# hkbharath/MARL-MASS

Measured on AMD Instinct MI355X. Metric: agent-steps/sec (whole node), MASS CBF shield on, 65536 envs x 8 CAVs, higher is better.
Workload: dtype f64

## Files before the change

marl-mass_amd/csrc/mm_kernels.hip:

```cpp
#include <hip/hip_runtime.h>
#include <math.h>
#include <stdio.h>
#include <string.h>

#include <type_traits>

#include "mm_device.h"
#include "mm_div.h"
#include "mm_handle.h"
#define MM_COUNTS_FN __host__ __device__ inline
#include "../../include/mm_counts.h"

using namespace mm;

struct DevCfg {
  int env_kind, shield, nsub, T, action_masking, auto_reset, obs_f64, N, E, debug_flags, n_hdv;
  double dt, collision_reward, high_speed_reward, headway_cost, headway_time, merging_lane_cost;
  double rs_lo, rs_hi, eta, tau;
  double inv_dt, rs_span, rs_ispan, rs_span2, rs_ispan2;
  int agent_reward;
  int steer_vel;
  int *err;
  int traffic_density, mixed_traffic, num_cav;
};
constexpr int kMetricsAccBit = 30;
#define MM_LATCH_QP_BOUNDS 1
#define MM_LATCH_BAD_ACTION 2
#define MM_LATCH_BAD_QP 4
#define MM_LATCH_INTERNAL 8
enum { MM_LW_STEP = 0, MM_LW_QP = 1, MM_LW_SHIELD = 2, MM_LW_COUNT = 3 };
struct DevState {
  double *F;
  uint8_t *B;
  int32_t *I;
  uint64_t *seeds;
  long long A;
  int E, N;
};

enum {
  SW_CPSI, SW_ACCN,
  SW_AX, SW_AY, SW_AH, SW_ACPSI, SW_AGVX, SW_ASTEER, SW_ASPSI,
  SW_BX, SW_BY, SW_BH, SW_BCPSI, SW_BGVX, SW_BSTEER, SW_BSPSI,
  SW_ACC,
  SW_F_COUNT
};
enum { SW_WPK, SW_APK, SW_BPK, SW_META, SW_RES, SW_CLS, SW_I_COUNT };
struct SweepBuf {
  double *F;
  int *I;
  uint8_t *order;
  uint8_t *envf;
  uint8_t *urgent;
  long long Ep;
  int N;
};
MM_DEV double &sw_f(const SweepBuf &sb, int f, int a, long long e) { return sb.F[((long long)f * sb.N + a) * sb.Ep + e]; }
MM_DEV int &sw_i(const SweepBuf &sb, int f, int a, long long e) { return sb.I[((long long)f * sb.N + a) * sb.Ep + e]; }

#ifndef MM_TU
#define MM_TU 0
#endif

#ifdef MM_STAMPS
#define MM_STAMP_WAVES (1 << 16)
__device__ unsigned long long g_stamps_w[MM_STAMP_WAVES * 16];
__device__ unsigned long long g_stamps_s[4096 * 8];
#define SSTAMP(k)                                                                        \
  do {                                                                                   \
    unsigned long long _t = __builtin_amdgcn_s_memtime();                                \
    if ((threadIdx.x & 63) == (k)) _t_acc += _t - _t_last;                               \
    _t_last = __builtin_amdgcn_s_memtime();                                              \
  } while (0)
#define SCOUNT(k) do { if ((threadIdx.x & 63) == (k)) _t_acc += 1; } while (0)
#define STAMP(k)                                                                         \
  do {                                                                                   \
    unsigned long long _t = __builtin_amdgcn_s_memtime();                                \
    if ((threadIdx.x & 63) == (k)) _t_acc += _t - _t_last;                               \
    _t_last = __builtin_amdgcn_s_memtime();                                              \
  } while (0)
#else
#define STAMP(k) do {} while (0)
#define SSTAMP(k) do {} while (0)
#define SCOUNT(k) do {} while (0)
#endif

template <int KIND> constexpr bool kIdm = KIND == MM_ENV_HDV_V1;

struct Veh {
  double x, y, h, v, tspeed;
  double act_steer, act_acc, safe_steer, safe_acc, gvx;
  double h1x, h1vx, h2x, h2vx;
  double sang;
  int lane, tlane, sidx, crashed, hl, flags, hist_len;
  int kind;
  bool present;
};

MM_DEV int lane_id() { return threadIdx.x & 63; }
MM_DEV double shfl_d(double v, int src) { return __shfl(v, src, 64); }
MM_DEV int shfl_i(int v, int src) { return __shfl(v, src, 64); }

template <int M>
MM_DEV int dppx_i(int v) {
  static_assert(M >= 1 && M <= 15, "xor mask within a 16-lane DPP row");
  if constexpr (M == 1) return __builtin_amdgcn_update_dpp(0, v, 0xB1, 0xF, 0xF, false);
  else if constexpr (M == 2) return __builtin_amdgcn_update_dpp(0, v, 0x4E, 0xF, 0xF, false);
  else if constexpr (M == 3) return __builtin_amdgcn_update_dpp(0, v, 0x1B, 0xF, 0xF, false);
  else if constexpr (M == 7) return __builtin_amdgcn_update_dpp(0, v, 0x141, 0xF, 0xF, false);
  else if constexpr (M == 8) return __builtin_amdgcn_update_dpp(0, v, 0x128, 0xF, 0xF, false);
  else if constexpr (M == 15) return __builtin_amdgcn_update_dpp(0, v, 0x140, 0xF, 0xF, false);
// ... 1036 lines not shown
      if (redo) {
#ifdef MM_STAMPS
        atomicAdd(&g_stamps_s[blockIdx.x % 4096 * 8 + 6], 1ull);
#endif
        s_redo[ln] = 0;
        reload_views();
        r = 0; dirty = (c.debug_flags & 1) != 0; nospec = true;
        phase = PH_SETUP;
      }
      continue;
    }
    if (__any(phase == PH_RUN)) {
      if (phase == PH_RUN) sing = mm_qp_bottom(&q, &rs) == 0;
    }
    SSTAMP(3);
  }
  if (e < c.E) sb.urgent[e] = slow_now ? 1 : 0;
#ifdef MM_STAMPS
  if ((threadIdx.x & 63) < 8 && blockIdx.x < 4096) g_stamps_s[blockIdx.x * 8 + (threadIdx.x & 63)] += _t_acc;
#endif
}

#ifndef MM_MIN_WAVES
#define MM_MIN_WAVES 2
#endif
#ifndef MM_NONE_WAVES
#define MM_NONE_WAVES 3
#endif
#ifndef MM_NONE_WIDE_G
#define MM_NONE_WIDE_G 99
#endif
#ifndef MM_IPM_WAVES
#define MM_IPM_WAVES 2
#endif
#ifndef MM_IPM_CAV_WAVES
#define MM_IPM_CAV_WAVES 2
#endif
#ifndef MM_IPM_WIDE_WAVES
#define MM_IPM_WIDE_WAVES 1
#endif
#ifndef MM_SPLIT_WAVES
#define MM_SPLIT_WAVES 2
#endif
template <int G, int SHIELD, bool MIXED>
#ifndef MM_GENERAL_NONE_WAVES
#define MM_GENERAL_NONE_WAVES 3
#endif
constexpr int step_min_waves(bool ipm = false) { return SHIELD == MM_SHIELD_NONE ? (G >= MM_NONE_WIDE_G ? 2 : (MIXED ? MM_GENERAL_NONE_WAVES : MM_NONE_WAVES)) : (ipm ? (G >= 6 ? MM_IPM_WIDE_WAVES : (MIXED ? MM_IPM_WAVES : MM_IPM_CAV_WAVES)) : MM_MIN_WAVES); }
template <int G, int KIND, int SHIELD, bool MIXED, bool IPM = false, bool TRACE = false, bool SPLIT = false>
#ifndef MM_STEP_BLOCK
#define MM_STEP_BLOCK 64
#endif
__global__ __launch_bounds__(MM_STEP_BLOCK, (SPLIT ? MM_SPLIT_WAVES : step_min_waves<G, SHIELD, MIXED>(IPM))) void step_kernel(DevCfg c, DevState st, const int32_t *__restrict__ actions,
                                                   MMStepOut out, double *metrics, SweepBuf sb, int kb) {
  constexpr bool IDM = kIdm<KIND>;
  constexpr bool LC = (KIND == MM_ENV_V1) || IDM;
  constexpr bool SHIELDED = LC && (SHIELD != MM_SHIELD_NONE);
  static_assert(!IDM || (MIXED && SHIELD == MM_SHIELD_NONE && !IPM && !SPLIT), "hdv-v1: general unshielded kernels only");
  constexpr bool MASS = (SHIELD == MM_SHIELD_MASS);
  static_assert(!IPM || SHIELDED, "the IPM mode lives in shielded kernels");
  static_assert(!SPLIT || IPM, "the split form exists for the interior-point kernels");
#ifdef MM_SERIAL_ALL
  constexpr bool kSerialOnly = true || IPM;
#else
#ifdef MM_SERIAL_MASS
  constexpr bool kSerialOnly = MIXED || MASS || IPM;
#else
  constexpr bool kSerialOnly = MIXED;
#endif
#endif
  constexpr bool kSine = SHIELDED && !SPLIT && !MIXED && !IPM && !kSerialOnly && kPow2<G> && G <= 8;
  static_assert(kPow2<G> || MM_STEP_BLOCK == 64, "rotation layouts: one wave per workgroup");
  const long long gtid = (long long)blockIdx.x * blockDim.x + threadIdx.x;
  constexpr int kTail = kPow2<G> ? 64 : (64 / G) * G;
  const bool tail = lane_id() >= kTail;
  const int gb = kPow2<G> ? (lane_id() & ~(G - 1)) : (tail ? kTail - G : lane_id() - lane_id() % G);
  const int a = kPow2<G> ? (int)(gtid % G) : lane_id() - gb;
  const long long e = kPow2<G> ? gtid / G : (tail ? (long long)st.E : (gtid >> 6) * (64 / G) + lane_id() / G);
  const bool valid = e < st.E && a < st.N;
  const long long i = e * st.N + a;
  const long long A = st.A;
  const double dt = c.dt;

#ifdef MM_STAMPS
  unsigned long long _t_last = __builtin_amdgcn_s_memtime(), _t_acc = 0;
#endif
  Veh v;
  const bool sv = MIXED && KIND == MM_ENV_V1 && c.steer_vel != 0;
  load_veh(st, i, valid, v, sv);
  int steps = 0, time = 0, n_merge = 0, episode = 0;
  if (e < st.E) {
    steps = st.I[MM_E_STEPS * st.E + e]; time = st.I[MM_E_TIME * st.E + e];
  }
  if (!MIXED && v.kind == 2) v.kind = 1;
  if (IDM && v.present) v.kind = 2;
  const bool hdv = MIXED && v.kind == 2;
  const bool ctrl = IDM ? v.present : (v.present && !hdv);
  const bool ctrl_x = IDM ? false : ctrl;
  int action = (!IDM && valid && ctrl) ? actions[i] : 1;
  if ((unsigned)action > 4u) {
    if (!SPLIT || kb == 0) atomicOr(c.err, MM_LATCH_BAD_ACTION);
    action = 1;
  }
  const unsigned present_bits = group_ballot<G>(v.present, gb);
  const unsigned ctrl_bits = group_ballot<G>(ctrl, gb);
  const int n_veh = __popc(present_bits), n_ctrl = __popc(ctrl_bits);
  if (!SPLIT || kb == 0) steps += 1;

  double cpsi = 1.0, spsi = 0.0;
  double st_t = __builtin_nan("");
  if (v.present) mmm_sincos(v.h, &spsi, &cpsi);
  int pk_self = v.lane;
  if (SHIELDED && v.present) pk_self = pose_code(v.lane, next_lane(v.lane, v.x, v.y), MASS ? corner_flags(v.x, v.y, spsi, cpsi, v.lane) : 0);

  enum { C_B = 0, C_H1X = 8, C_H1VX, C_H2X, C_H2VX, C_SSTEER, C_SACC, C_TSPEED, C_A = 15, C_GU0 = 23, C_GU1 = 24, C_PRE = 25, C_MSGW = 29 };
  constexpr bool kMailbox = G <= 8 || !kPow2<G>;
  constexpr bool kPackMsg = !kPow2<G>;
  constexpr int kColdB = kMailbox ? (kPackMsg ? 29 : 30) : 25;
  constexpr bool kRoomy = false;
  constexpr int C_CPSI = kColdB + G - 1, C_GVX = C_CPSI + 1;
  constexpr int kColdN = !SHIELDED ? 15 : (kSerialOnly ? 23 : kColdB + G - 1 + (kRoomy ? 2 : 0));
  static_assert(kColdN * MM_STEP_BLOCK * 8 >= (MM_STEP_BLOCK / 64) * 64 * 30 * 4, "the obs staging must fit in the cold slots");
  __shared__ double s_cold[kColdN][MM_STEP_BLOCK];
  const int tid = threadIdx.x;
  auto cold_i = [&](int slot, int col) -> int & { return ((int *)&s_cold[slot][col])[0]; };
  if (LC) {
    s_cold[C_H1X][tid] = v.h1x; s_cold[C_H1VX][tid] = v.h1vx; s_cold[C_H2X][tid] = v.h2x; s_cold[C_H2VX][tid] = v.h2vx;
    s_cold[C_SSTEER][tid] = v.safe_steer; s_cold[C_SACC][tid] = v.safe_acc;
  }
  s_cold[C_TSPEED][tid] = v.tspeed;
  if constexpr (kRoomy) { s_cold[C_CPSI][tid] = cpsi; s_cold[C_GVX][tid] = v.gvx; }
  auto CPSI = [&]() -> double { if constexpr (kRoomy) return s_cold[C_CPSI][tid]; else return cpsi; };
  auto GVX = [&]() -> double { if constexpr (kRoomy) return s_cold[C_GVX][tid]; else return v.gvx; };
  bool env_active = IDM ? n_veh > 0 : n_ctrl > 0;
  if constexpr (SPLIT) {
    if (kb > 0) env_active = e < st.E && sb.envf[e] != 0;
  }
  STAMP(0);
  const int k_lo = SPLIT ? (kb > 0 ? kb - 1 : 0) : 0, k_hi = SPLIT ? (kb < c.nsub ? kb : c.nsub - 1) : c.nsub - 1;
  for (int k = k_lo; k <= k_hi; k++) {
    const bool head = !SPLIT || k == kb, tail = !SPLIT || k != kb;
    const bool live = env_active && v.present;
    QpTrace qt = {0, __builtin_nan(""), __builtin_nan(""), __builtin_nan(""), __builtin_nan(""),
                  __builtin_nan(""), __builtin_nan(""), __builtin_nan("")};
    int rank = 0;
    if ((SHIELDED || MIXED) && head) {
      for_partners<G>([&](auto mc) {
        constexpr int m = decltype(mc)::value;
        double px = px_d<m, G>(v.x, a);
        bool pp = px_i<m, G>((int)live, a) != 0;
        rank += (pp && (px > v.x || (px == v.x && pidx<m, G>(a) < a))) ? 1 : 0;
      });
    }
    if (head) v.tspeed = s_cold[C_TSPEED][tid];
    if (live && !hdv && head) {
      if (time % c.nsub == 0) hl_act<KIND>(v, action);
    }
    const int tl_pre = v.tlane;
    if (live && !hdv && head) controlled_act<!MIXED, kSine>(v, -1, sv, st_t);
    if (head) s_cold[C_TSPEED][tid] = v.tspeed;
    if constexpr (MIXED) { STAMP(1); }
    if constexpr (MIXED) {
      if (head && __any(hdv && live)) {
        const bool acting = hdv && live && !v.crashed;
        double koff = 0.0, koff_obst = 0.0;
        if (__any(acting && v.lane == MM_LANE_KB0)) {
// ... 772 lines not shown
  }
  if (valid) {
    if (out.agents_rewards) out.agents_rewards[i] = ctrl ? local : 0;
    if (out.regional_rewards) out.regional_rewards[i] = ctrl ? regional : 0;
    if (out.agents_dones) out.agents_dones[i] = ctrl ? (uint8_t)(v.crashed || steps >= c.T || v.x < 0) : 1;
    if (out.crashed) out.crashed[i] = v.present ? (uint8_t)v.crashed : 0;
    if (out.agents_info) {
      out.agents_info[i * 3 + 0] = v.present ? v.x : 0;
      out.agents_info[i * 3 + 1] = v.present ? v.y : 0;
      out.agents_info[i * 3 + 2] = v.present ? v.v : 0;
    }
  }
  if (e < st.E && a == 0 && env_ok) {
    if (out.reward) out.reward[e] = reward;
    if (out.done) out.done[e] = (uint8_t)done;
    if (out.average_speed) out.average_speed[e] = avg_speed;
    if (out.traffic_speed) out.traffic_speed[e] = traffic_speed;
    if (out.min_headway) out.min_headway[e] = min_headway;
    if (out.merge_percent) out.merge_percent[e] = merge_pct;
  }
  STAMP(10);
  if (metrics) {
    static_assert(MM_STEP_BLOCK % 64 == 0, "whole waves per workgroup");
    const bool lead = e < st.E && a == 0 && env_ok;
    const double mv[8] = {lead ? reward : 0.0, (lead && done && crashed_bits) ? 1.0 : 0.0, lead ? avg_speed : 0.0,
                          lead ? traffic_speed : 0.0, lead ? 1.0 : 0.0, (lead && done) ? merge_pct : 0.0,
                          (lead && done) ? 1.0 : 0.0, lead ? min_headway : INFINITY};
    if (a == 0) {
#pragma unroll
      for (int k = 0; k < 8; k++) s_cold[C_B + k][tid] = mv[k];
    }
    __builtin_amdgcn_fence(__ATOMIC_RELEASE, "wavefront");
    __builtin_amdgcn_wave_barrier();
    __builtin_amdgcn_fence(__ATOMIC_ACQUIRE, "wavefront");
    const int ln = lane_id();
    if (ln < 8) {
      const int slot = C_B + ln, base = tid - ln;
      double acc = ln == 7 ? INFINITY : 0.0;
#pragma unroll
      for (int j = 0; j < 64 / G; j++) {
        const double x = s_cold[slot][base + j * G];
        acc = ln == 7 ? fmin(acc, x) : acc + x;
      }
      double *row = metrics + (gtid >> 6) * 8;
      if ((c.debug_flags >> kMetricsAccBit) & 1) {
        if (ln == 7) (void)unsafeAtomicMin(&row[7], acc);
        else (void)unsafeAtomicAdd(&row[ln], acc);
      } else {
        row[ln] = acc;
      }
    }
  }
  STAMP(15);
  if (c.auto_reset && done) {
    const uint64_t seed = st.seeds[e];
    Veh nv;
    memset(&nv, 0, sizeof nv);
    int nm = 0;
    int nc = n_ctrl, nh = n_veh - n_ctrl;
    if constexpr (IDM) { nc = 0; nh = n_veh; }
    episode_counts<KIND>(c, seed, (uint32_t)episode, nc, nh);
    const bool spawn = valid && (c.traffic_density > 0 ? a < nc + nh : v.present);
    if (spawn) nm = spawn_vehicle(nv, a, nc, nh, seed, (uint32_t)episode);
    if (c.traffic_density > 0 && valid) {
      if (!spawn) {
        if (v.present) {
          Veh z;
          memset(&z, 0, sizeof z);
          store_veh(st, i, z, true);
        }
        v.present = false; v.kind = 0;
      }
      st.B[MM_B_KIND * A + i] = spawn ? (uint8_t)nv.kind : (uint8_t)0;
    }
    if (spawn) {
      v = nv;
      spsi = 0.0; cpsi = 1.0;
      s_cold[C_H1X][tid] = v.h1x; s_cold[C_H1VX][tid] = v.h1vx; s_cold[C_H2X][tid] = v.h2x; s_cold[C_H2VX][tid] = v.h2vx;
      s_cold[C_SSTEER][tid] = v.safe_steer; s_cold[C_SACC][tid] = v.safe_acc; s_cold[C_TSPEED][tid] = v.tspeed;
    }
    n_merge = shfl_i(nm, gb);
    steps = 0; time = 0; episode += 1;
  }
  if (valid && v.present) {
    if (LC) {
      v.h1x = s_cold[C_H1X][tid]; v.h1vx = s_cold[C_H1VX][tid]; v.h2x = s_cold[C_H2X][tid]; v.h2vx = s_cold[C_H2VX][tid];
      if (!hdv) { v.safe_steer = s_cold[C_SSTEER][tid]; v.safe_acc = s_cold[C_SACC][tid]; }
    }
    v.tspeed = s_cold[C_TSPEED][tid];
    store_veh(st, i, v, sv);
  }
  if (e < st.E && a == 0) {
    st.I[MM_E_STEPS * st.E + e] = steps; st.I[MM_E_TIME * st.E + e] = time;
    st.I[MM_E_N_MERGE * st.E + e] = n_merge; st.I[MM_E_EPISODE * st.E + e] = episode;
  }
  STAMP(11);
  __syncthreads();
  STAMP(14);
  const double sc_h[2] = {spsi, cpsi};
  observe<G, KIND, true>(c, v, a, gb, i, valid, out.obs, out.action_mask, (float *)&s_cold[0][0], sc_h);
  STAMP(12);
#ifdef MM_STAMPS
  {
    const long long wv = gtid >> 6;
    if ((threadIdx.x & 63) < 16 && wv < MM_STAMP_WAVES) g_stamps_w[wv * 16 + (threadIdx.x & 63)] += _t_acc;
  }
#endif
}

template <int G, int KIND>
__global__ __launch_bounds__(256) void reset_kernel(DevCfg c, DevState st, int mode, const uint8_t *env_mask,
                                                    const uint64_t *seeds_in, void *obs, uint8_t *avail) {
  const long long gtid = (long long)blockIdx.x * blockDim.x + threadIdx.x;
  const long long e = gtid / G;
  const int a = (int)(gtid % G);
  const int gb = lane_id() & ~(G - 1);
  const bool valid = e < st.E && a < st.N;
  const long long i = e * st.N + a;
  const bool selected = e < st.E && mode != 2 && (!env_mask || env_mask[e]);
  Veh v;
  load_veh(st, i, valid, v);
  if (kIdm<KIND> && v.present) v.kind = 2;
  if (selected) {
    int steps = 0, time = 0, n_merge = 0, episode = st.I[MM_E_EPISODE * st.E + e];
    if (mode == 0) {
      if (seeds_in && a == 0) st.seeds[e] = seeds_in[e];
      const uint64_t seed = seeds_in ? seeds_in[e] : st.seeds[e];
      int nm = 0;
      int nc = st.N - c.n_hdv, nh = c.n_hdv;
      if (kIdm<KIND>) { nc = 0; nh = st.N; }
      episode_counts<KIND>(c, seed, (uint32_t)episode, nc, nh);
      if (valid) {
        if (a < nc + nh) nm = spawn_vehicle(v, a, nc, nh, seed, (uint32_t)episode);
        else {
          const bool was = v.present;
          memset(&v, 0, sizeof v);
          if (was) store_veh(st, i, v, true);
          v.hl = MM_HL_NONE;
        }
        st.B[MM_B_KIND * st.A + i] = (uint8_t)v.kind;
      }
      n_merge = shfl_i(nm, gb);
      episode += 1;
// ... 151 lines not shown
    return;
  }
  double hc = hh[0];
  if (m == 4 && hh[3] < hc) hc = hh[3];
  double d;
  if (a > 0) d = fmin(0.0, hc / a);
  else if (a < 0) d = fmax(0.0, hc / a);
  else d = 0.0;
  d = fmin(fmax(d, -hh[2]), hh[1]);
  const double s = a * d - hc;
  u[k * 3 + 0] = d; u[k * 3 + 1] = 0.0; u[k * 3 + 2] = s > 0 ? s : 0.0;
  if (status) status[k] = MM_QPS_OPTIMAL;
}

#endif

#if MM_TU <= 1
constexpr int kFlushWaves = 256;
__global__ __launch_bounds__(256) void metrics_flush_kernel(double *partial, long long waves, double *metrics, int reset) {
  __shared__ double s_p[32][8];
  const int k = threadIdx.x & 7, r = threadIdx.x >> 3;
  const long long w0 = (long long)blockIdx.x * kFlushWaves;
  double x[kFlushWaves / 32];
#pragma unroll
  for (int j = 0; j < kFlushWaves / 32; j++) {
    const long long w = w0 + r + 32 * j;
    x[j] = w < waves ? partial[w * 8 + k] : (k == 7 ? INFINITY : 0.0);
    if (reset && w < waves) partial[w * 8 + k] = k == 7 ? INFINITY : 0.0;
  }
  double acc = k == 7 ? INFINITY : 0.0;
#pragma unroll
  for (int j = 0; j < kFlushWaves / 32; j++) acc = k == 7 ? fmin(acc, x[j]) : acc + x[j];
  if (reset == 2) return;
  s_p[r][k] = acc;
  __syncthreads();
  if (threadIdx.x < 8) {
    double t = k == 7 ? INFINITY : 0.0;
    for (int j = 0; j < 32; j++) t = k == 7 ? fmin(t, s_p[j][k]) : t + s_p[j][k];
    if (k == 7) atomic_min_d(&metrics[7], t);
    else atomicAdd(&metrics[k], t);
  }
}
#endif

static int group_size(int N) { return N <= 2 ? 2 : (N <= 4 ? 4 : (N <= 8 ? 8 : 16)); }

struct MMHandle_ : MMHandleHead {
  double *metrics;
  double *metrics_partial;
  int metrics_deferred;
  int *dev_err;
  SweepBuf sweep;
  void *sweep_mem;
  int n_simd;
  char err[256];
};
static bool needs_general(const MMHandle_ *h) {
  return h->cfg.env_kind == MM_ENV_HDV_V1 || h->cfg.n_hdv > 0 || (h->cfg.traffic_density > 0 && h->cfg.mixed_traffic != 0) ||
         (h->cfg.env_kind == MM_ENV_V1 && h->cfg.lateral_control == MM_LATERAL_STEER_VEL);
}
static bool steps_split(const MMHandle_ *h) {
  if (!(h->cfg.env_kind == MM_ENV_V1 && h->cfg.shield != MM_SHIELD_NONE && h->cfg.qp_solver == MM_QP_IPM)) return false;
  if (h->cfg.debug_flags & 4) return false;
  if (h->cfg.debug_flags & 8) return true;
  const int g = h->N <= 2 ? 2 : (h->N <= 4 ? 4 : (h->N <= 8 ? 8 : 16));
  return (long long)h->E * g / 64 > (g >= 8 ? 1ll : 2ll) * (h->n_simd > 0 ? h->n_simd : 1024);
}

static long long step_launch_waves(const MMHandle h) {
  const long long threads = (long long)h->E * group_size(h->N);
  return (threads + MM_STEP_BLOCK - 1) / MM_STEP_BLOCK * (MM_STEP_BLOCK / 64);
}
static int step_group(const MMHandle h) {
  const int g = group_size(h->N);
#if defined(MM_ONLY_G)
  (void)g;
  return MM_ONLY_G;
#elif defined(MM_NO_LANES)
  return g;
#else
  if (h->cfg.debug_flags & 2) return g;
  if (h->N == 5 || h->N == 6) return 6;
  if (h->N >= 9 && h->N <= 12) return 12;
  return g;
#endif
}
static long long step_launch_waves_now(const MMHandle h) {
  const int g = step_group(h);
  if ((g & (g - 1)) == 0) return step_launch_waves(h);
  const long long epw = 64 / g;
  return (h->E + epw - 1) / epw;
}
#if MM_TU <= 1
static uint64_t align256(uint64_t x) { return (x + 255u) & ~(uint64_t)255u; }

extern "C" int32_t mm_abi_version(void) { return MM_ABI_VERSION; }

const MMHandleHead *mm_handle_head(MMHandle h) { return h; }

extern "C" int32_t mm_state_layout(int32_t E, int32_t N, MMStateLayout *out) {
  if (!out || E <= 0 || N <= 0 || N > MM_MAX_AGENTS) return MM_ERR_INVALID_ARG;
  uint64_t A = (uint64_t)E * (uint64_t)N, off = 0;
  out->f64_offset = off; off = align256(off + A * 8u * MM_F_COUNT);
  out->u8_offset = off; off = align256(off + A * MM_B_COUNT);
  out->env_offset = off; off = align256(off + (uint64_t)E * 4u * MM_E_COUNT);
  out->seed_offset = off; off = align256(off + (uint64_t)E * 8u);
  out->total_bytes = off;
  return MM_OK;
}

static int check_cfg(const MMConfig *c, int N, char *err) {
  if (!c || c->abi_version != MM_ABI_VERSION) { snprintf(err, 256, "ABI version mismatch"); return MM_ERR_INVALID_ARG; }
  if (c->env_kind != MM_ENV_V0 && c->env_kind != MM_ENV_V1 && c->env_kind != MM_ENV_HDV_V1) { snprintf(err, 256, "unknown env_kind %d", c->env_kind); return MM_ERR_INVALID_ARG; }
  if (c->env_kind == MM_ENV_HDV_V1) {
    if (c->shield != MM_SHIELD_NONE) { snprintf(err, 256, "merge-multi-agent-hdv-v1 has no controlled vehicle: shield must be none, got %d", c->shield); return MM_ERR_INVALID_ARG; }
    if (c->lateral_control != MM_LATERAL_STEER) { snprintf(err, 256, "merge-multi-agent-hdv-v1 has no controlled vehicle: lateral_control must be steer"); return MM_ERR_INVALID_ARG; }
    if (c->n_hdv != 0) { snprintf(err, 256, "merge-multi-agent-hdv-v1: every vehicle is an HDV, n_hdv must be 0 (got %d)", c->n_hdv); return MM_ERR_INVALID_ARG; }
  }
  if (c->shield < MM_SHIELD_NONE || c->shield > MM_SHIELD_MASS) { snprintf(err, 256, "Undefined safety_type:%d", c->shield); return MM_ERR_INVALID_ARG; }
  if (c->policy_frequency <= 0 || c->simulation_frequency < c->policy_frequency ||
      c->simulation_frequency / c->policy_frequency > 3) { snprintf(err, 256, "unsupported frequencies"); return MM_ERR_INVALID_ARG; }
  if (N > 12) { snprintf(err, 256, "N=%d exceeds the 6+6 spawn slots", N); return MM_ERR_INVALID_ARG; }
  if (c->env_kind != MM_ENV_HDV_V1 && (c->n_hdv < 0 || c->n_hdv >= N)) { snprintf(err, 256, "n_hdv=%d must leave at least one controlled vehicle of N=%d", c->n_hdv, N); return MM_ERR_INVALID_ARG; }
  if (c->qp_solver != MM_QP_EXACT && c->qp_solver != MM_QP_IPM) { snprintf(err, 256, "unknown qp_solver %d", c->qp_solver); return MM_ERR_INVALID_ARG; }
  if (mm_counts_check(c, N, 0, err, 256)) return MM_ERR_INVALID_ARG;
  return MM_OK;
}

static hipError_t ensure_sweep(MMHandle_ *h) {
  if (h->sweep_mem || !steps_split(h)) return hipSuccess;
  const uint64_t Ep = ((uint64_t)h->E + 63u) & ~(uint64_t)63u, N = (uint64_t)h->N;
  const uint64_t bF = align256(Ep * N * 8u * SW_F_COUNT), bI = align256(Ep * N * 4u * SW_I_COUNT), bO = align256(Ep * N), bE = 2 * align256(Ep);
  unsigned char *m = nullptr;
  hipError_t rc = hipMalloc((void **)&m, bF + bI + bO + bE);
  if (rc != hipSuccess) return rc;
  rc = hipMemset(m, 0, bF + bI + bO + bE);
  if (rc != hipSuccess) { (void)hipFree(m); return rc; }
  h->sweep_mem = m;
  h->sweep.F = (double *)m; h->sweep.I = (int *)(m + bF); h->sweep.order = m + bF + bI; h->sweep.envf = m + bF + bI + bO;
  h->sweep.urgent = h->sweep.envf + align256(Ep);
  h->sweep.Ep = (long long)Ep; h->sweep.N = h->N;
  return hipSuccess;
}

static thread_local char g_create_err[256] = "null handle";
void mm_set_thread_error(const char *text) { snprintf(g_create_err, sizeof g_create_err, "%s", text); }
struct DeviceGuard {
  int prev = -1;
  hipError_t rc;
  explicit DeviceGuard(int device) {
    if (hipGetDevice(&prev) != hipSuccess) prev = -1;
    rc = hipSetDevice(device);
  }
  ~DeviceGuard() { if (prev >= 0) (void)hipSetDevice(prev); }
};
static int hip_fail(MMHandle h, hipError_t e, const char *what) {
  snprintf(h->err, sizeof h->err, "%s: %s", what, hipGetErrorString(e));
  return MM_ERR_DEVICE;
}

extern "C" int32_t mm_create(const MMConfig *cfg, int32_t E, int32_t N, int32_t device, void *state,
                             uint64_t state_bytes, int64_t first_env, MMHandle *out) {
  if (!out || !state) return MM_ERR_INVALID_ARG;
  MMHandle h = (MMHandle)calloc(1, sizeof(struct MMHandle_));
  snprintf(h->err, sizeof h->err, "mm_create: E, N, the state buffer (size, 256-byte alignment) or the configuration is invalid");
  if (mm_state_layout(E, N, &h->lay) != MM_OK || state_bytes < h->lay.total_bytes ||
      ((uintptr_t)state & 255u) || check_cfg(cfg, N, h->err) != MM_OK) {
    snprintf(g_create_err, sizeof g_create_err, "%s", h->err);
    free(h);
    return MM_ERR_INVALID_ARG;
  }
  h->err[0] = 0;
  h->cfg = *cfg; h->E = E; h->N = N; h->device = device; h->state = (unsigned char *)state;
  h->first_env = first_env;
  uint64_t *tmp = (uint64_t *)malloc((size_t)E * 8u);
  for (int64_t e = 0; e < E; e++) tmp[e] = cfg->seed + (uint64_t)(first_env + e);
  DeviceGuard dg(device);
  hipError_t rc = dg.rc;
  if (rc == hipSuccess) {
    int cus = 0;
    rc = hipDeviceGetAttribute(&cus, hipDeviceAttributeMultiprocessorCount, device);
    h->n_simd = 4 * cus;
  }
  if (rc == hipSuccess) rc = hipMemcpy(h->state + h->lay.seed_offset, tmp, (size_t)E * 8u, hipMemcpyHostToDevice);
  free(tmp);
  if (rc == hipSuccess) rc = hipMalloc((void **)&h->dev_err, MM_LW_COUNT * sizeof(int));
  if (rc == hipSuccess) rc = hipMemset(h->dev_err, 0, MM_LW_COUNT * sizeof(int));
  if (rc == hipSuccess) rc = ensure_sweep(h);
  if (rc != hipSuccess) { if (h->dev_err) (void)hipFree(h->dev_err); free(h); return MM_ERR_DEVICE; }
  *out = h;
  return MM_OK;
}
extern "C" int32_t mm_destroy(MMHandle h) {
  if (!h) return MM_OK;
  DeviceGuard dg(h->device);
  hipError_t rc = dg.rc;
  if (rc == hipSuccess) rc = hipDeviceSynchronize();
  if (h->dev_err) (void)hipFree(h->dev_err);
  if (h->metrics_partial) (void)hipFree(h->metrics_partial);
  if (h->sweep_mem) (void)hipFree(h->sweep_mem);
  free(h);
  return rc == hipSuccess ? MM_OK : MM_ERR_DEVICE;
}
static int poll_latch(MMHandle h, int word, MMStream stream) {
  int bits = 0;
  DeviceGuard dg(h->device);
  hipError_t rc = dg.rc;
  if (rc == hipSuccess) rc = hipStreamSynchronize((hipStream_t)stream);
  if (rc == hipSuccess) rc = hipMemcpy(&bits, h->dev_err + word, sizeof bits, hipMemcpyDeviceToHost);
  if (rc == hipSuccess && bits) rc = hipMemset(h->dev_err + word, 0, sizeof(int));
  if (rc != hipSuccess) return hip_fail(h, rc, "error poll");
  if (!bits) return MM_OK;
  snprintf(h->err, sizeof h->err, "%s%s%s%s",
           (bits & MM_LATCH_QP_BOUNDS) ? "Error in QP. Invalid accceleration; " : "",
           (bits & MM_LATCH_BAD_ACTION) ? "an action is outside 0..4; " : "",
           (bits & MM_LATCH_BAD_QP) ? "mm_shield_qp: G is not of the form get_G builds (cbf.py:288-304,386-403); " : "",
           (bits & MM_LATCH_INTERNAL) ? "internal: a kernel loop guard fired; " : "");
  if (bits & MM_LATCH_INTERNAL) return MM_ERR_DEVICE;
  if (bits & MM_LATCH_QP_BOUNDS) return MM_ERR_QP_BOUNDS;
  return MM_ERR_INVALID_ARG;
}
static void launch_metrics_flush(MMHandle h, hipStream_t s, int reset) {
  const long long waves = reset ? step_launch_waves(h) : step_launch_waves_now(h);
  hipLaunchKernelGGL(metrics_flush_kernel, dim3((unsigned)((waves + kFlushWaves - 1) / kFlushWaves)), dim3(256), 0, s,
                     h->metrics_partial, waves, h->metrics, reset);
}
extern "C" int32_t mm_flush_metrics(MMHandle h, MMStream stream) {
  if (!h) return MM_ERR_INVALID_ARG;
  if (!h->metrics_deferred || !h->metrics) return MM_OK;
  DeviceGuard dg(h->device);
  if (dg.rc != hipSuccess) return hip_fail(h, dg.rc, "metrics flush");
  launch_metrics_flush(h, (hipStream_t)stream, 1);
  const hipError_t rc = hipGetLastError();
  return rc == hipSuccess ? MM_OK : hip_fail(h, rc, "metrics flush");
}
extern "C" int32_t mm_defer_metrics(MMHandle h, int32_t deferred, MMStream stream) {
  if (!h) return MM_ERR_INVALID_ARG;
  if (deferred && !h->metrics) {
    snprintf(h->err, sizeof h->err, "mm_defer_metrics: no metrics buffer (mm_set_metrics_buffer first)");
    return MM_ERR_INVALID_ARG;
  }
  if ((deferred != 0) == (h->metrics_deferred != 0)) return MM_OK;
  DeviceGuard dg(h->device);
  if (dg.rc != hipSuccess) return hip_fail(h, dg.rc, "mm_defer_metrics");
  if (deferred) {
    const long long waves = step_launch_waves(h);
    hipLaunchKernelGGL(metrics_flush_kernel, dim3((unsigned)((waves + kFlushWaves - 1) / kFlushWaves)), dim3(256), 0,
                       (hipStream_t)stream, h->metrics_partial, waves, (double *)nullptr, 2);
    h->metrics_deferred = 1;
  } else {
    launch_metrics_flush(h, (hipStream_t)stream, 1);
    h->metrics_deferred = 0;
  }
  const hipError_t rc = hipGetLastError();
  return rc == hipSuccess ? MM_OK : hip_fail(h, rc, "mm_defer_metrics");
}
extern "C" int32_t mm_poll_errors(MMHandle h, MMStream stream) {
  if (!h) return MM_ERR_INVALID_ARG;
  const int frc = mm_flush_metrics(h, stream);
  if (frc != MM_OK) return frc;
  return poll_latch(h, MM_LW_STEP, stream);
}
extern "C" int32_t mm_set_config(MMHandle h, const MMConfig *cfg) {
  if (!h) return MM_ERR_INVALID_ARG;
  int rc = check_cfg(cfg, h->N, h->err);
  if (rc != MM_OK) return rc;
  h->cfg = *cfg;
  DeviceGuard dg(h->device);
  hipError_t hrc = dg.rc;
  if (hrc == hipSuccess) hrc = ensure_sweep(h);
  return hrc == hipSuccess ? MM_OK : hip_fail(h, hrc, "hand-off planes of the split interior-point step");
}
extern "C" int32_t mm_set_metrics_buffer(MMHandle h, double *metrics) {
  if (!h) return MM_ERR_INVALID_ARG;
  if (metrics && !h->metrics_partial) {
    const long long waves = step_launch_waves(h);
    DeviceGuard dg(h->device);
    hipError_t rc = dg.rc;
    if (rc == hipSuccess) rc = hipMalloc((void **)&h->metrics_partial, (size_t)waves * 8 * sizeof(double));
    if (rc != hipSuccess) return hip_fail(h, rc, "metrics partial buffer");
  }
  if (h->metrics_deferred && h->metrics && metrics != h->metrics) {
    DeviceGuard dg(h->device);
    hipError_t rc = dg.rc;
    if (rc == hipSuccess) { launch_metrics_flush(h, (hipStream_t)0, 1); rc = hipGetLastError(); }
    if (rc == hipSuccess) rc = hipStreamSynchronize((hipStream_t)0);
    if (rc != hipSuccess) return hip_fail(h, rc, "metrics flush before the buffer switch");
  }
  h->metrics = metrics;
  if (!metrics) h->metrics_deferred = 0;
  return MM_OK;
}
extern "C" const char *mm_last_error(MMHandle h) { return h ? h->err : g_create_err; }
#endif

static DevCfg dev_cfg(const MMHandle h) {
  const MMConfig &c = h->cfg;
  DevCfg d;
  d.env_kind = c.env_kind; d.shield = c.env_kind == MM_ENV_V1 ? c.shield : MM_SHIELD_NONE;
  d.nsub = c.simulation_frequency / c.policy_frequency; d.T = c.duration * c.policy_frequency;
  d.action_masking = c.action_masking; d.auto_reset = c.auto_reset; d.obs_f64 = c.obs_f64; d.N = h->N; d.E = h->E;
  d.debug_flags = (c.debug_flags & ~(1 << kMetricsAccBit)) | (h->metrics_deferred ? (1 << kMetricsAccBit) : 0); d.n_hdv = c.n_hdv;
  d.dt = 1.0 / c.simulation_frequency;
  d.collision_reward = c.collision_reward; d.high_speed_reward = c.high_speed_reward;
  d.headway_cost = c.headway_cost; d.headway_time = c.headway_time; d.merging_lane_cost = c.merging_lane_cost;
  d.rs_lo = c.reward_speed_lo; d.rs_hi = c.reward_speed_hi; d.eta = c.cbf_eta; d.tau = c.cbf_tau;
  d.inv_dt = 1.0 / d.dt; d.rs_span = d.rs_hi - d.rs_lo; d.rs_ispan = 1.0 / d.rs_span;
  d.rs_span2 = (d.rs_lo + (d.rs_hi - d.rs_lo) / 2) - d.rs_lo; d.rs_ispan2 = 1.0 / d.rs_span2;
  d.agent_reward = c.env_kind == MM_ENV_V1 ? c.agent_reward : 0;
  d.steer_vel = (c.env_kind == MM_ENV_V1 && c.lateral_control == MM_LATERAL_STEER_VEL) ? 1 : 0;
  d.err = h->dev_err + MM_LW_STEP;
  d.traffic_density = c.traffic_density; d.mixed_traffic = c.mixed_traffic; d.num_cav = c.num_cav;
  return d;
}
static DevState dev_state(const MMHandle h) {
  DevState s;
  s.F = (double *)(h->state + h->lay.f64_offset); s.B = h->state + h->lay.u8_offset;
  s.I = (int32_t *)(h->state + h->lay.env_offset); s.seeds = (uint64_t *)(h->state + h->lay.seed_offset);
  s.A = (long long)h->E * h->N; s.E = h->E; s.N = h->N;
  return s;
}
void mm_launch_reset_idm(MMHandle h, int mode, const uint8_t *mask, const uint64_t *seeds, void *obs, uint8_t *avail, hipStream_t s);
void mm_launch_step_idm(MMHandle h, int g, const MMStepOut *out, hipStream_t s);
#if MM_TU <= 1 || MM_TU == 8
// ... 6 lines not shown
                     seeds, obs, avail);
}
#endif
#if MM_TU <= 1
template <int G>
static void launch_reset_g(MMHandle h, int mode, const uint8_t *mask, const uint64_t *seeds, void *obs,
                           uint8_t *avail, hipStream_t s) {
  if (h->cfg.env_kind == MM_ENV_V1) launch_reset_t<G, MM_ENV_V1>(h, mode, mask, seeds, obs, avail, s);
  else launch_reset_t<G, MM_ENV_V0>(h, mode, mask, seeds, obs, avail, s);
}
static int launch_reset(MMHandle h, int mode, const uint8_t *mask, const uint64_t *seeds, void *obs,
                        uint8_t *avail, MMStream stream) {
  hipStream_t s = (hipStream_t)stream;
  if (h->cfg.env_kind == MM_ENV_HDV_V1) mm_launch_reset_idm(h, mode, mask, seeds, obs, avail, s);
  else
#ifdef MM_ONLY_G
  launch_reset_g<MM_ONLY_G>(h, mode, mask, seeds, obs, avail, s);
#else
  switch (group_size(h->N)) {
    case 2: launch_reset_g<2>(h, mode, mask, seeds, obs, avail, s); break;
    case 4: launch_reset_g<4>(h, mode, mask, seeds, obs, avail, s); break;
    case 8: launch_reset_g<8>(h, mode, mask, seeds, obs, avail, s); break;
    default: launch_reset_g<16>(h, mode, mask, seeds, obs, avail, s); break;
  }
#endif
  hipError_t rc = hipGetLastError();
  return rc == hipSuccess ? MM_OK : hip_fail(h, rc, "reset launch");
}

extern "C" int32_t mm_reset(MMHandle h, const uint8_t *env_mask, const uint64_t *seeds, void *obs,
                            uint8_t *avail, MMStream stream) {
  if (!h) return MM_ERR_INVALID_ARG;
  if (mm_counts_check(&h->cfg, h->N, 1, h->err, sizeof h->err)) return MM_ERR_INVALID_ARG;
  return launch_reset(h, 0, env_mask, seeds, obs, avail, stream);
}
extern "C" int32_t mm_init_from_kinematics(MMHandle h, const uint8_t *env_mask, MMStream stream) {
  if (!h) return MM_ERR_INVALID_ARG;
  return launch_reset(h, 1, env_mask, nullptr, nullptr, nullptr, stream);
}
extern "C" int32_t mm_observe(MMHandle h, void *obs, uint8_t *avail, MMStream stream) {
  if (!h) return MM_ERR_INVALID_ARG;
  return launch_reset(h, 2, nullptr, nullptr, obs, avail, stream);
}

#endif

template <int G, int KIND, int SHIELD, bool MIXED, bool IPM = false>
static void launch_step_t(MMHandle h, const int32_t *actions, const MMStepOut *out, hipStream_t s) {
  const long long threads = (long long)h->E * G;
  const unsigned grid = kPow2<G> ? (unsigned)((threads + MM_STEP_BLOCK - 1) / MM_STEP_BLOCK)
                                 : (unsigned)((h->E + 64 / G - 1) / (64 / G));
  if (out->trace)
    hipLaunchKernelGGL((step_kernel<G, KIND, SHIELD, MIXED, IPM, true>), dim3(grid), dim3(MM_STEP_BLOCK), 0, s, dev_cfg(h), dev_state(h),
                       actions, *out, h->metrics ? h->metrics_partial : nullptr, h->sweep, 0);
  else
    hipLaunchKernelGGL((step_kernel<G, KIND, SHIELD, MIXED, IPM, false>), dim3(grid), dim3(MM_STEP_BLOCK), 0, s, dev_cfg(h), dev_state(h),
                       actions, *out, h->metrics ? h->metrics_partial : nullptr, h->sweep, 0);
}
#if MM_TU == 0 || MM_TU == 6 || MM_TU == 7
template <int G, int SHIELD, bool MIXED>
static void launch_split_gs(MMHandle h, const int32_t *actions, const MMStepOut *out, hipStream_t s) {
  const long long threads = (long long)h->E * G;
  const unsigned grid = kPow2<G> ? (unsigned)((threads + MM_STEP_BLOCK - 1) / MM_STEP_BLOCK)
                                 : (unsigned)((h->E + 64 / G - 1) / (64 / G));
  const DevCfg dc = dev_cfg(h);
  const DevState ds = dev_state(h);
  const unsigned sgrid = (unsigned)((h->E + 63) / 64);
  constexpr bool MASS = SHIELD == MM_SHIELD_MASS;
  for (int kb = 0; kb <= dc.nsub; kb++) {
    hipLaunchKernelGGL((step_kernel<G, MM_ENV_V1, SHIELD, MIXED, true, true, true>), dim3(grid), dim3(MM_STEP_BLOCK), 0, s, dc, ds, actions,
                       *out, h->metrics ? h->metrics_partial : nullptr, h->sweep, kb);
    if (kb == dc.nsub) break;
    auto pad = [](size_t used) { return (unsigned)(used < 40960 ? 40960 - used : 0); };
    constexpr size_t kPerVeh = 6 * 64 * sizeof(double) + 3 * 64 * sizeof(unsigned short);
    if (h->N <= 4) hipLaunchKernelGGL((sweep_kernel<4, MASS, MIXED>), dim3(sgrid), dim3(64), pad(4 * kPerVeh + 5632), s, dc, ds, h->sweep, kb, out->trace);
    else if (h->N <= 8) hipLaunchKernelGGL((sweep_kernel<8, MASS, MIXED>), dim3(sgrid), dim3(64), pad(8 * kPerVeh + 5632), s, dc, ds, h->sweep, kb, out->trace);
    else if (h->N <= 11) hipLaunchKernelGGL((sweep_kernel<11, MASS, MIXED>), dim3(sgrid), dim3(64), pad(11 * kPerVeh + 1024), s, dc, ds, h->sweep, kb, out->trace);
    else hipLaunchKernelGGL((sweep_kernel<12, MASS, MIXED>), dim3(sgrid), dim3(64), pad(12 * kPerVeh + 1024), s, dc, ds, h->sweep, kb, out->trace);
  }
}
template <bool MIXED>
static void launch_split_all(MMHandle h, int g, const int32_t *actions, const MMStepOut *out, hipStream_t s) {
  const bool mass = h->cfg.shield == MM_SHIELD_MASS;
  switch (g) {
#define MM_SPLIT_CASE(GG) case GG: if (mass) launch_split_gs<GG, MM_SHIELD_MASS, MIXED>(h, actions, out, s); else launch_split_gs<GG, MM_SHIELD_HSS, MIXED>(h, actions, out, s); break;
#ifdef MM_ONLY_G
    MM_SPLIT_CASE(MM_ONLY_G)
#else
    MM_SPLIT_CASE(2) MM_SPLIT_CASE(4) MM_SPLIT_CASE(6) MM_SPLIT_CASE(8) MM_SPLIT_CASE(12) MM_SPLIT_CASE(16)
#endif
#undef MM_SPLIT_CASE
    default: break;
  }
}
#if MM_TU == 7
void mm_launch_step_split_general(MMHandle h, int g, const int32_t *actions, const MMStepOut *out, hipStream_t s) { launch_split_all<true>(h, g, actions, out, s); }
#elif MM_TU == 6
void mm_launch_step_split_general(MMHandle h, int g, const int32_t *actions, const MMStepOut *out, hipStream_t s);
void mm_launch_step_split(MMHandle h, int g, const int32_t *actions, const MMStepOut *out, hipStream_t s) {
  if (needs_general(h)) mm_launch_step_split_general(h, g, actions, out, s);
  else launch_split_all<false>(h, g, actions, out, s);
}
#else
static void mm_launch_step_split(MMHandle h, int g, const int32_t *actions, const MMStepOut *out, hipStream_t s) {
#ifdef MM_ONLY_MIXED
  launch_split_all<MM_ONLY_MIXED>(h, g, actions, out, s);
#else
  if (needs_general(h)) launch_split_all<true>(h, g, actions, out, s);
  else launch_split_all<false>(h, g, actions, out, s);
#endif
}
#endif
#endif
template <int G, bool MIXED>
static void launch_step_m(MMHandle h, const int32_t *actions, const MMStepOut *out, hipStream_t s) {
#ifdef MM_ONLY_SHIELD
  launch_step_t<G, MM_ENV_V1, MM_ONLY_SHIELD, MIXED>(h, actions, out, s);
  return;
#endif
  if (h->cfg.env_kind == MM_ENV_V0) { launch_step_t<G, MM_ENV_V0, MM_SHIELD_NONE, MIXED>(h, actions, out, s); return; }
  switch (h->cfg.shield) {
    case MM_SHIELD_HSS: launch_step_t<G, MM_ENV_V1, MM_SHIELD_HSS, MIXED>(h, actions, out, s); break;
    case MM_SHIELD_MASS: launch_step_t<G, MM_ENV_V1, MM_SHIELD_MASS, MIXED>(h, actions, out, s); break;
    default: launch_step_t<G, MM_ENV_V1, MM_SHIELD_NONE, MIXED>(h, actions, out, s);
// ... 71 lines not shown
    case 4: launch_step_m<4, true>(h, actions, out, s); break;
    case 8: launch_step_m<8, true>(h, actions, out, s); break;
    default: launch_step_m<16, true>(h, actions, out, s); break;
  }
}
#elif MM_TU == 3
void mm_launch_step_ipm(MMHandle h, const int32_t *actions, const MMStepOut *out, hipStream_t s) {
  switch (group_size(h->N)) {
    case 2: launch_step_ipm_g<2>(h, actions, out, s); break;
    case 4: launch_step_ipm_g<4>(h, actions, out, s); break;
    case 8: launch_step_ipm_g<8>(h, actions, out, s); break;
    default: launch_step_ipm_g<16>(h, actions, out, s); break;
  }
}
#else
template <int G>
static void launch_step_g(MMHandle h, const int32_t *actions, const MMStepOut *out, hipStream_t s) {
#ifdef MM_ONLY_MIXED
#ifdef MM_ONLY_IPM
  launch_step_t<G, MM_ENV_V1, MM_ONLY_SHIELD, MM_ONLY_MIXED, true>(h, actions, out, s);
#else
  launch_step_m<G, MM_ONLY_MIXED>(h, actions, out, s);
#endif
#else
  const bool shielded = h->cfg.env_kind == MM_ENV_V1 && h->cfg.shield != MM_SHIELD_NONE;
  if (shielded && h->cfg.qp_solver == MM_QP_IPM)
#if MM_TU == 1
    mm_launch_step_ipm(h, actions, out, s);
#else
    launch_step_ipm_g<G>(h, actions, out, s);
#endif
  else if (needs_general(h))
#if MM_TU == 1
    mm_launch_step_general(h, actions, out, s);
#else
    launch_step_m<G, true>(h, actions, out, s);
#endif
  else launch_step_m<G, false>(h, actions, out, s);
#endif
}

extern "C" int32_t mm_step(MMHandle h, const int32_t *actions, const MMStepOut *out, MMStream stream) {
  if (!h || !out || (!actions && h->cfg.env_kind != MM_ENV_HDV_V1)) return MM_ERR_INVALID_ARG;
  hipStream_t s = (hipStream_t)stream;
  if (out->trace) {
    hipError_t rc = hipMemsetAsync(out->trace, 0xFF, (size_t)3 * MM_T_COUNT * h->E * h->N * sizeof(double), s);
    if (rc != hipSuccess) return hip_fail(h, rc, "trace memset");
  }
  if (h->cfg.env_kind == MM_ENV_HDV_V1) {
    mm_launch_step_idm(h, step_group(h), out, s);
  } else if (steps_split(h)) {
    if (!h->sweep_mem) { snprintf(h->err, sizeof h->err, "mm_step: the hand-off planes of the split interior-point step are missing"); return MM_ERR_DEVICE; }
    mm_launch_step_split(h, step_group(h), actions, out, s);
  } else
#ifdef MM_ONLY_G
  launch_step_g<MM_ONLY_G>(h, actions, out, s);
#else
  switch (step_group(h)) {
    case 2: launch_step_g<2>(h, actions, out, s); break;
    case 4: launch_step_g<4>(h, actions, out, s); break;
    case 8: launch_step_g<8>(h, actions, out, s); break;
    case 6: case 12: mm_launch_step_lanes(h, step_group(h), actions, out, s); break;
    default: launch_step_g<16>(h, actions, out, s); break;
  }
#endif
  if (h->metrics && !h->metrics_deferred) launch_metrics_flush(h, s, 0);
  hipError_t rc = hipGetLastError();
  return rc == hipSuccess ? MM_OK : hip_fail(h, rc, "step launch");
}


template <int G, bool IPM>
static void launch_shield_gi(MMHandle h, const double *as, const double *aa, double *ss, double *sa, uint8_t *stt,
                             double *mg, double *hw, hipStream_t s) {
  const long long threads = (long long)h->E * G;
  const unsigned grid = (unsigned)((threads + 255) / 256);
  const int sh = h->cfg.env_kind == MM_ENV_V1 ? h->cfg.shield : MM_SHIELD_NONE;
  DevCfg dc = dev_cfg(h);
  dc.err = h->dev_err + MM_LW_SHIELD;
  if (sh == MM_SHIELD_MASS)
    hipLaunchKernelGGL((shield_kernel<G, MM_SHIELD_MASS, IPM>), dim3(grid), dim3(256), 0, s, dc, dev_state(h), as, aa, ss, sa, stt, mg, hw);
  else if (sh == MM_SHIELD_HSS)
    hipLaunchKernelGGL((shield_kernel<G, MM_SHIELD_HSS, IPM>), dim3(grid), dim3(256), 0, s, dc, dev_state(h), as, aa, ss, sa, stt, mg, hw);
  else
    hipLaunchKernelGGL((shield_kernel<G, MM_SHIELD_NONE, false>), dim3(grid), dim3(256), 0, s, dc, dev_state(h), as, aa, ss, sa, stt, mg, hw);
}
template <int G>
static void launch_shield_g(MMHandle h, const double *as, const double *aa, double *ss, double *sa, uint8_t *stt,
                            double *mg, double *hw, hipStream_t s) {
  if (h->cfg.qp_solver == MM_QP_IPM) launch_shield_gi<G, true>(h, as, aa, ss, sa, stt, mg, hw, s);
  else launch_shield_gi<G, false>(h, as, aa, ss, sa, stt, mg, hw, s);
}
extern "C" int32_t mm_shield_actions(MMHandle h, const double *act_steer, const double *act_acc, double *safe_steer,
                                     double *safe_acc, uint8_t *status, double *margin, double *headway, MMStream stream) {
  if (!h || !act_steer || !act_acc || !safe_steer || !safe_acc) return MM_ERR_INVALID_ARG;
  hipStream_t s = (hipStream_t)stream;
#ifdef MM_ONLY_G
  launch_shield_g<MM_ONLY_G>(h, act_steer, act_acc, safe_steer, safe_acc, status, margin, headway, s);
#else
  switch (group_size(h->N)) {
    case 2: launch_shield_g<2>(h, act_steer, act_acc, safe_steer, safe_acc, status, margin, headway, s); break;
    case 4: launch_shield_g<4>(h, act_steer, act_acc, safe_steer, safe_acc, status, margin, headway, s); break;
    case 8: launch_shield_g<8>(h, act_steer, act_acc, safe_steer, safe_acc, status, margin, headway, s); break;
    default: launch_shield_g<16>(h, act_steer, act_acc, safe_steer, safe_acc, status, margin, headway, s); break;
  }
#endif
// ... 323 lines not shown
```

Before: 2.263 billion.

## Carry per-vehicle sin/cos and pose code across steps in a device buffer

Adds a persistent per-agent buffer storing the end-of-step pose (x, y, heading bits), sin/cos of heading and the packed pose code. On the next step the kernel checks, per wave, whether every present vehicle's state bit-matches the cached key. If so it reuses the cached trig and pose code instead of recomputing mmm_sincos and corner_flags. This trades extra global loads and stores (six values per agent per step) for skipping transcendental and geometry work. The gain is unclear because the kernel may be memory-bound.

Measured after the change: 2.300 billion, median of 6. 1.6% higher.

```diff
diff --git a/marl-mass_amd/csrc/mm_kernels.hip b/marl-mass_amd/csrc/mm_kernels.hip
--- a/marl-mass_amd/csrc/mm_kernels.hip
+++ b/marl-mass_amd/csrc/mm_kernels.hip
@@ -57,6 +57,13 @@
 };
 MM_DEV double &sw_f(const SweepBuf &sb, int f, int a, long long e) { return sb.F[((long long)f * sb.N + a) * sb.Ep + e]; }
 MM_DEV int &sw_i(const SweepBuf &sb, int f, int a, long long e) { return sb.I[((long long)f * sb.N + a) * sb.Ep + e]; }
+
+enum { PB_SIN, PB_COS, PB_KX, PB_KY, PB_KH, PB_F_COUNT };
+constexpr int kPoseWritten = 0x200;
+struct PoseBuf {
+  double *F;
+  int *code;
+};
 
 #ifndef MM_TU
 #define MM_TU 0
@@ -1199,7 +1206,7 @@
 #define MM_STEP_BLOCK 64
 #endif
 __global__ __launch_bounds__(MM_STEP_BLOCK, (SPLIT ? MM_SPLIT_WAVES : step_min_waves<G, SHIELD, MIXED>(IPM))) void step_kernel(DevCfg c, DevState st, const int32_t *__restrict__ actions,
-                                                   MMStepOut out, double *metrics, SweepBuf sb, int kb) {
+                                                   MMStepOut out, double *metrics, SweepBuf sb, int kb, PoseBuf pb) {
   constexpr bool IDM = kIdm<KIND>;
   constexpr bool LC = (KIND == MM_ENV_V1) || IDM;
   constexpr bool SHIELDED = LC && (SHIELD != MM_SHIELD_NONE);
@@ -1217,6 +1224,10 @@
 #endif
 #endif
   constexpr bool kSine = SHIELDED && !SPLIT && !MIXED && !IPM && !kSerialOnly && kPow2<G> && G <= 8;
+#ifndef MM_CARRY_POSE
+#define MM_CARRY_POSE 1
+#endif
+  constexpr bool kCarry = kSine && MM_CARRY_POSE != 0;
   static_assert(kPow2<G> || MM_STEP_BLOCK == 64, "rotation layouts: one wave per workgroup");
   const long long gtid = (long long)blockIdx.x * blockDim.x + threadIdx.x;
   constexpr int kTail = kPow2<G> ? 64 : (64 / G) * G;
@@ -1234,8 +1245,18 @@
 #endif
   Veh v;
   const bool sv = MIXED && KIND == MM_ENV_V1 && c.steer_vel != 0;
+  int steps = 0, time = 0, n_merge = 0, episode = 0;
+  int car_code = 0;
+  long long car_kx = 0, car_ky = 0, car_kh = 0;
+  double car_s = 0.0, car_c = 1.0;
+  if constexpr (kCarry) {
+    if (valid) {
+      car_kx = __double_as_longlong(pb.F[PB_KX * A + i]); car_ky = __double_as_longlong(pb.F[PB_KY * A + i]);
+      car_kh = __double_as_longlong(pb.F[PB_KH * A + i]);
+      car_s = pb.F[PB_SIN * A + i]; car_c = pb.F[PB_COS * A + i]; car_code = pb.code[i];
+    }
+  }
   load_veh(st, i, valid, v, sv);
-  int steps = 0, time = 0, n_merge = 0, episode = 0;
   if (e < st.E) {
     steps = st.I[MM_E_STEPS * st.E + e]; time = st.I[MM_E_TIME * st.E + e];
   }
@@ -1256,9 +1277,18 @@
 
   double cpsi = 1.0, spsi = 0.0;
   double st_t = __builtin_nan("");
-  if (v.present) mmm_sincos(v.h, &spsi, &cpsi);
   int pk_self = v.lane;
-  if (SHIELDED && v.present) pk_self = pose_code(v.lane, next_lane(v.lane, v.x, v.y), MASS ? corner_flags(v.x, v.y, spsi, cpsi, v.lane) : 0);
+  bool carried = false;
+  if constexpr (kCarry) {
+    const bool hit = car_kx == __double_as_longlong(v.x) && car_ky == __double_as_longlong(v.y) && car_kh == __double_as_longlong(v.h) &&
+                     (car_code >> 8) == ((kPoseWritten >> 8) | (MASS ? 1 : 0)) && (car_code & 7) == v.lane;
+    carried = !__any(v.present && !hit);
+    if (carried && v.present) { spsi = car_s; cpsi = car_c; pk_self = car_code & 0xFF; }
+  }
+  if (!carried) {
+    if (v.present) mmm_sincos(v.h, &spsi, &cpsi);
+    if (SHIELDED && v.present) pk_self = pose_code(v.lane, next_lane(v.lane, v.x, v.y), MASS ? corner_flags(v.x, v.y, spsi, cpsi, v.lane) : 0);
+  }
 
   enum { C_B = 0, C_H1X = 8, C_H1VX, C_H2X, C_H2VX, C_SSTEER, C_SACC, C_TSPEED, C_A = 15, C_GU0 = 23, C_GU1 = 24, C_PRE = 25, C_MSGW = 29 };
   constexpr bool kMailbox = G <= 8 || !kPow2<G>;
@@ -2137,6 +2167,7 @@
     }
   }
   STAMP(15);
+  if constexpr (kCarry) { car_s = spsi; car_c = cpsi; }
   if (c.auto_reset && done) {
     const uint64_t seed = st.seeds[e];
     Veh nv;
@@ -2161,6 +2192,10 @@
     if (spawn) {
       v = nv;
       spsi = 0.0; cpsi = 1.0;
+      if constexpr (kCarry) {
+        mmm_sincos(v.h, &car_s, &car_c);
+        pk_self = pose_code(v.lane, next_lane(v.lane, v.x, v.y), MASS ? corner_flags(v.x, v.y, car_s, car_c, v.lane) : 0);
+      }
       s_cold[C_H1X][tid] = v.h1x; s_cold[C_H1VX][tid] = v.h1vx; s_cold[C_H2X][tid] = v.h2x; s_cold[C_H2VX][tid] = v.h2vx;
       s_cold[C_SSTEER][tid] = v.safe_steer; s_cold[C_SACC][tid] = v.safe_acc; s_cold[C_TSPEED][tid] = v.tspeed;
     }
@@ -2174,6 +2209,11 @@
     }
     v.tspeed = s_cold[C_TSPEED][tid];
     store_veh(st, i, v, sv);
+    if constexpr (kCarry) {
+      pb.F[PB_KX * A + i] = v.x; pb.F[PB_KY * A + i] = v.y; pb.F[PB_KH * A + i] = v.h;
+      pb.F[PB_SIN * A + i] = car_s; pb.F[PB_COS * A + i] = car_c;
+      pb.code[i] = (pk_self & 0xFF) | (MASS ? 0x100 : 0) | kPoseWritten;
+    }
   }
   if (e < st.E && a == 0) {
     st.I[MM_E_STEPS * st.E + e] = steps; st.I[MM_E_TIME * st.E + e] = time;
@@ -2431,6 +2471,8 @@
   int *dev_err;
   SweepBuf sweep;
   void *sweep_mem;
+  PoseBuf pose;
+  void *pose_mem;
   int n_simd;
   char err[256];
 };
@@ -2522,6 +2564,21 @@
   return hipSuccess;
 }
 
+static bool carries_pose(const MMHandle_ *h) { return h->cfg.env_kind == MM_ENV_V1 && h->cfg.shield != MM_SHIELD_NONE; }
+static hipError_t ensure_pose(MMHandle_ *h) {
+  if (h->pose_mem || !carries_pose(h)) return hipSuccess;
+  const uint64_t A = (uint64_t)h->E * (uint64_t)h->N;
+  const uint64_t bF = align256(A * 8u * PB_F_COUNT), bI = align256(A * 4u);
+  unsigned char *m = nullptr;
+  hipError_t rc = hipMalloc((void **)&m, bF + bI);
+  if (rc != hipSuccess) return rc;
+  rc = hipMemset(m, 0, bF + bI);
+  if (rc != hipSuccess) { (void)hipFree(m); return rc; }
+  h->pose_mem = m;
+  h->pose.F = (double *)m; h->pose.code = (int *)(m + bF);
+  return hipSuccess;
+}
+
 static thread_local char g_create_err[256] = "null handle";
 void mm_set_thread_error(const char *text) { snprintf(g_create_err, sizeof g_create_err, "%s", text); }
 struct DeviceGuard {
@@ -2566,7 +2623,13 @@
   if (rc == hipSuccess) rc = hipMalloc((void **)&h->dev_err, MM_LW_COUNT * sizeof(int));
   if (rc == hipSuccess) rc = hipMemset(h->dev_err, 0, MM_LW_COUNT * sizeof(int));
   if (rc == hipSuccess) rc = ensure_sweep(h);
-  if (rc != hipSuccess) { if (h->dev_err) (void)hipFree(h->dev_err); free(h); return MM_ERR_DEVICE; }
+  if (rc == hipSuccess) rc = ensure_pose(h);
+  if (rc != hipSuccess) {
+    if (h->dev_err) (void)hipFree(h->dev_err);
+    if (h->sweep_mem) (void)hipFree(h->sweep_mem);
+    free(h);
+    return MM_ERR_DEVICE;
+  }
   *out = h;
   return MM_OK;
 }
@@ -2578,6 +2641,7 @@
   if (h->dev_err) (void)hipFree(h->dev_err);
   if (h->metrics_partial) (void)hipFree(h->metrics_partial);
   if (h->sweep_mem) (void)hipFree(h->sweep_mem);
+  if (h->pose_mem) (void)hipFree(h->pose_mem);
   free(h);
   return rc == hipSuccess ? MM_OK : MM_ERR_DEVICE;
 }
@@ -2648,7 +2712,9 @@
   DeviceGuard dg(h->device);
   hipError_t hrc = dg.rc;
   if (hrc == hipSuccess) hrc = ensure_sweep(h);
-  return hrc == hipSuccess ? MM_OK : hip_fail(h, hrc, "hand-off planes of the split interior-point step");
+  if (hrc != hipSuccess) return hip_fail(h, hrc, "hand-off planes of the split interior-point step");
+  hrc = ensure_pose(h);
+  return hrc == hipSuccess ? MM_OK : hip_fail(h, hrc, "carried pose planes");
 }
 extern "C" int32_t mm_set_metrics_buffer(MMHandle h, double *metrics) {
   if (!h) return MM_ERR_INVALID_ARG;
@@ -2761,10 +2827,10 @@
                                  : (unsigned)((h->E + 64 / G - 1) / (64 / G));
   if (out->trace)
     hipLaunchKernelGGL((step_kernel<G, KIND, SHIELD, MIXED, IPM, true>), dim3(grid), dim3(MM_STEP_BLOCK), 0, s, dev_cfg(h), dev_state(h),
-                       actions, *out, h->metrics ? h->metrics_partial : nullptr, h->sweep, 0);
+                       actions, *out, h->metrics ? h->metrics_partial : nullptr, h->sweep, 0, h->pose);
   else
     hipLaunchKernelGGL((step_kernel<G, KIND, SHIELD, MIXED, IPM, false>), dim3(grid), dim3(MM_STEP_BLOCK), 0, s, dev_cfg(h), dev_state(h),
-                       actions, *out, h->metrics ? h->metrics_partial : nullptr, h->sweep, 0);
+                       actions, *out, h->metrics ? h->metrics_partial : nullptr, h->sweep, 0, h->pose);
 }
 #if MM_TU == 0 || MM_TU == 6 || MM_TU == 7
 template <int G, int SHIELD, bool MIXED>
@@ -2778,7 +2844,7 @@
   constexpr bool MASS = SHIELD == MM_SHIELD_MASS;
   for (int kb = 0; kb <= dc.nsub; kb++) {
     hipLaunchKernelGGL((step_kernel<G, MM_ENV_V1, SHIELD, MIXED, true, true, true>), dim3(grid), dim3(MM_STEP_BLOCK), 0, s, dc, ds, actions,
-                       *out, h->metrics ? h->metrics_partial : nullptr, h->sweep, kb);
+                       *out, h->metrics ? h->metrics_partial : nullptr, h->sweep, kb, h->pose);
     if (kb == dc.nsub) break;
     auto pad = [](size_t used) { return (unsigned)(used < 40960 ? 40960 - used : 0); };
     constexpr size_t kPerVeh = 6 * 64 * sizeof(double) + 3 * 64 * sizeof(unsigned short);
@@ -2956,6 +3022,9 @@
   } else if (steps_split(h)) {
     if (!h->sweep_mem) { snprintf(h->err, sizeof h->err, "mm_step: the hand-off planes of the split interior-point step are missing"); return MM_ERR_DEVICE; }
     mm_launch_step_split(h, step_group(h), actions, out, s);
+  } else if (carries_pose(h) && !h->pose_mem) {
+    snprintf(h->err, sizeof h->err, "mm_step: the carried pose planes are missing");
+    return MM_ERR_DEVICE;
   } else
 #ifdef MM_ONLY_G
   launch_step_g<MM_ONLY_G>(h, actions, out, s);
```
